# liuhx02/YourEditableAvatar

Hardware: AMD Instinct MI355X
Metric: rasterized fragments/sec (fwd+bwd) @500k Gaussians 1080p (higher is better)
Workload: dtype f32

## Files before the change

youreditableavatar_amd/csrc/tgs_api.hip:

```cpp
#include "tgs_device.hpp"
#include "../../include/tgs_raster.h"
#include "../../include/tgs_raster_testing.h"

#include <cstdarg>
#include <cstdio>
#include <cstring>

namespace tgs {
void launch_preprocess_fwd(hipStream_t, const FwdIn&, const CamParams&, const GeomState&, const ImgState&);
void launch_preprocess_fwd_batch(hipStream_t, const FwdIn&, const FwdViews&);
void launch_scan(hipStream_t, const GeomState&, const ImgState&, uint32_t nblocks, uint32_t T, uint32_t sort_cap, unsigned long long r_capacity,
                 uint32_t tile_bound, uint32_t heavy_bound, uint32_t mid_bound, Meta* host_meta, int light);
void launch_bin_count(hipStream_t, int P, const GeomState&, const ImgState&, uint32_t gx, uint32_t T);
void launch_scatter(hipStream_t, int P, const GeomState&, const ImgState&, const BinState&, uint32_t gx, uint32_t T);
void launch_tile_sort(hipStream_t, const GeomState&, const ImgState&, const BinState&, uint32_t gx, uint32_t T, uint64_t r_bound, const Meta* m,
                      uint32_t sort_cap, uint32_t tile_bound, uint32_t heavy_bound, uint32_t mid_bound);
void launch_render_fwd(hipStream_t, const ImgState&, const BinState&, int W, int H, uint32_t gx, uint32_t T, const Meta* m, const float* bg,
                       float* out_color, uint32_t tile_bound, uint32_t mid_bound, int light);
void launch_mark_visible(hipStream_t, int P, const float* means3D, const float* view, uint8_t* present);
void launch_alpha(hipStream_t, const ImgState&, size_t N, float* out_alpha);
void launch_render_bwd(hipStream_t, const ImgState&, const BinState&, int W, int H, uint32_t gx, uint32_t tiles, const float* bg, const float* dL_dpix,
                       const float* dL_dalpha, bool deterministic, uint32_t mid_tiles, int light, uint32_t T);
void launch_preprocess_bwd(hipStream_t, const BwdIn&, const CamParams&, const GeomState&, const BinState&);
void launch_preprocess_bwd_batch(hipStream_t, const BwdIn&, const BatchViews&);
// ... 906 lines not shown

int tgs_mark_visible(void* stream, int P, const float* means3D, const float* viewmatrix, const float* projmatrix, uint8_t* present)
{
    hipStream_t st = (hipStream_t)stream;
    g_err[0] = 0;
    (void)projmatrix;
    if (P == 0) return TGS_OK;
    if (P < 0 || !means3D || !viewmatrix || !present) return fail(TGS_ERR_INVALID, "bad arguments");
    launch_mark_visible(st, P, means3D, viewmatrix, present);
    hipError_t e = hipGetLastError();
    if (e != hipSuccess) return fail(TGS_ERR_HIP, "mark_visible: %s", hipGetErrorString(e));
    return TGS_OK;
}

int64_t tgs_state_field(void* stream, const char* field, int P, int width, int height, int64_t R, int has_sh, int has_scale_rot,
                        const void* geom_buffer, const void* binning_buffer, const void* img_buffer, void* dst, size_t dst_bytes)
{
    hipStream_t st = (hipStream_t)stream;
    g_err[0] = 0;
    const ViewArgs v{nullptr, width, height, nullptr, nullptr, nullptr, 0.f, 0.f};
    const size_t N = v.N(), T = v.T();
    const FrameBuffers fb = carve_frame(GeomShape{(size_t)P, has_sh != 0, has_scale_rot != 0}, v, R, geom_buffer, binning_buffer, img_buffer);
    const GeomState& g = fb.g; const ImgState& s = fb.s; const BinState& b = fb.b;
    const void* src = nullptr; size_t count = 0, esz = 4, stride = 0, rows = 0;
    if (!strcmp(field, "n_contrib")) { src = s.n_contrib; count = N; }
    else if (!strcmp(field, "final_T")) { src = s.final_T; count = N; }
    else if (!strcmp(field, "ranges")) { src = s.ranges; count = 2 * T; }
    else if (!strcmp(field, "means2D")) { src = g.pack; count = 2 * (size_t)P; esz = 8; stride = 64; rows = (size_t)P; }
    else if (!strcmp(field, "depths")) { src = g.depth; count = (size_t)P; }
    else if (!strcmp(field, "conic_opacity")) { src = (const char*)g.pack + 8; count = 4 * (size_t)P; esz = 16; stride = 64; rows = (size_t)P; }
    else if (!strcmp(field, "rgb")) { src = (const char*)g.pack + 24; count = 3 * (size_t)P; esz = 12; stride = 64; rows = (size_t)P; }
    else if (!strcmp(field, "tiles_touched")) { src = g.tiles_touched; count = (size_t)P; }
    else if (!strcmp(field, "tile_order")) { src = s.tile_order; count = T; }
    else if (!strcmp(field, "stamps")) { src = s.stamps; count = 8 * T; esz = 8; }
    else if (!strcmp(field, "block_masks")) { src = (const char*)b.recC + 4; count = (size_t)R; esz = 4; stride = 8; rows = (size_t)R; }
    else if (!strcmp(field, "quad_masks")) { src = b.qmask; count = (size_t)R; esz = 8; }
    else if (!strcmp(field, "point_list")) { src = b.keys; count = (size_t)R; esz = 4; stride = 8; rows = (size_t)R; }
    else return fail(TGS_ERR_INVALID, "unknown field %s", field);
    const size_t total = stride ? rows * esz : count * esz;
    if (dst_bytes < total) return fail(TGS_ERR_INVALID, "dst too small for %s", field);
    if (count == 0) return 0;
    if (stride) HIP_TRY(hipMemcpy2DAsync(dst, esz, src, stride, esz, rows, hipMemcpyDeviceToDevice, st));
    else HIP_TRY(hipMemcpyAsync(dst, src, total, hipMemcpyDeviceToDevice, st));
    return (int64_t)count;
}

}
```

youreditableavatar_amd/csrc/tgs_device.hpp:

```cpp
#pragma once
#include <hip/hip_runtime.h>
#include <cstdlib>
#include <stddef.h>
#include <stdint.h>

namespace tgs {

constexpr int TILE = 16;
constexpr int TILE_PIX = TILE * TILE;
constexpr int WAVE = 64;
constexpr int PRE_BLOCK = 256;
constexpr uint32_t SORT_LDS_CAP = 8192;
constexpr int COOP_TILES = 64;
constexpr int RANK_TILES = 4;
constexpr int SLAB_ROW = 3;
#ifndef TGS_BIN_WGS_MAX
#define TGS_BIN_WGS_MAX 256
#endif
constexpr int BIN_WGS_MAX = TGS_BIN_WGS_MAX;
constexpr int BIN_THREADS = 1024;
constexpr uint32_t BIN_LDS_TILES = 24576;

struct Meta {
    unsigned long long R;
    uint32_t max_count;
    uint32_t n_overflow;
    uint32_t error;
    uint32_t n_nonempty;
    uint32_t n_heavy;
    uint32_t n_mid;
    uint32_t pad[8];
};

constexpr uint32_t META_ERR_CAPACITY = 2u;
constexpr uint32_t META_ERR_TILE_BOUND = 4u;

struct ScanAux {
    uint32_t hist[40];
    uint32_t cursor[40];
    uint32_t done;
    uint32_t pad[47];
};
static_assert(sizeof(ScanAux) == 512, "ScanAux: 128 words, cleared by the first 128 threads of a block");

struct GeomState {
    float4* pack;
    uint2* live;
    float* depth;
    uint8_t* clamped;
    ushort4* rect;
    uint32_t* tiles_touched;
    uint32_t* offsets;
    uint32_t* block_sums;
    uint32_t* block_flags;
};
struct ImgState {
    Meta* meta;
    ScanAux* aux;
    uint2* ranges;
    uint32_t* tile_count;
    uint32_t* bin_table;
    uint32_t* ovf_tiles;
    uint32_t* tile_order;
    uint4* tile_desc;
    uint4* light_desc;
    float* final_T;
    uint32_t* n_contrib;
    unsigned long long* stamps;
};
struct BinState {
    unsigned long long* keys;
    uint32_t* tile_of;
    float4* recA;
    float4* recB;
    float2* recC;
    uint32_t* slot;
    uint2* qmask;
    float4* slab;
};

template <typename T>
__host__ __device__ inline void carve(char*& p, T*& out, size_t count)
{
    uintptr_t a = (reinterpret_cast<uintptr_t>(p) + 255) & ~uintptr_t(255);
    out = reinterpret_cast<T*>(a);
    p = reinterpret_cast<char*>(out + count);
}
__host__ __device__ inline size_t n_blocks(size_t P) { return (P + PRE_BLOCK - 1) / PRE_BLOCK; }

__host__ __device__ inline size_t geom_carve(GeomState& g, char* base, size_t P, bool has_sh, bool has_scale_rot)
{
    char* p = base;
    (void)has_sh; (void)has_scale_rot;
    carve(p, g.pack, 4 * P); carve(p, g.live, P); carve(p, g.depth, P);
    carve(p, g.clamped, P); carve(p, g.rect, P); carve(p, g.tiles_touched, P); carve(p, g.offsets, P);
    carve(p, g.block_sums, n_blocks(P) + 1); carve(p, g.block_flags, n_blocks(P) + 1);
    return (size_t)(p - base) + 256;
}
__host__ __device__ inline size_t img_carve(ImgState& s, char* base, size_t N, size_t T)
{
    char* p = base;
    carve(p, s.meta, 1); carve(p, s.aux, 1); carve(p, s.ranges, T); carve(p, s.tile_count, T); carve(p, s.bin_table, (size_t)BIN_WGS_MAX * T);
    carve(p, s.ovf_tiles, T); carve(p, s.tile_order, T); carve(p, s.tile_desc, T); carve(p, s.light_desc, T);
    carve(p, s.final_T, N); carve(p, s.n_contrib, N);
    carve(p, s.stamps, 8 * T);
    return (size_t)(p - base) + 256;
}
__host__ __device__ inline size_t bin_carve(BinState& b, char* base, size_t R)
{
    char* p = base;
    carve(p, b.keys, R); carve(p, b.tile_of, R); carve(p, b.recA, R); carve(p, b.recB, R); carve(p, b.recC, R); carve(p, b.slot, R); carve(p, b.qmask, R); carve(p, b.slab, (size_t)SLAB_ROW * R);
    return (size_t)(p - base) + 256;
}

int set_error(int code, const char* msg);
int hip_status(const char* what);

#ifdef __HIPCC__
#define TGS_DPP_ADD(v, ctrl, rowmask)                                                                      \
    v += __builtin_bit_cast(float, __builtin_amdgcn_update_dpp(0, __builtin_bit_cast(int, v), ctrl, rowmask, 0xf, false))

__device__ __forceinline__ float wave_sum(float v)
{
    TGS_DPP_ADD(v, 0xB1, 0xf);
    TGS_DPP_ADD(v, 0x4E, 0xf);
    TGS_DPP_ADD(v, 0x141, 0xf);
    TGS_DPP_ADD(v, 0x140, 0xf);
    TGS_DPP_ADD(v, 0x142, 0xa);
    TGS_DPP_ADD(v, 0x143, 0xc);
// ... 706 lines not shown
```

youreditableavatar_amd/csrc/tgs_forward.hip:

```cpp
#include "tgs_device.hpp"

namespace tgs {

__device__ __forceinline__ float conic_min_on_edge(float dfix, float lo, float hi, float Pfix, float Pvar, float B, float mB_over_Pvar)
{
    const float t = fminf(hi, fmaxf(lo, dfix * mB_over_Pvar));
    return 0.5f * (Pfix * dfix * dfix + Pvar * t * t) + B * dfix * t;
}

__device__ __forceinline__ unsigned long long quadrant_mask(float2 xy, float4 co, uint32_t tx, uint32_t ty)
{
    const float o255 = 255.0f * co.w;
    if (o255 < 0.999f) return 0ull;
    const float tau = (fmaxf(__logf(o255), 0.f) + 0.01f) * 1.001f;
    const float A = co.x, B = co.y, Cc = co.z;
    const float det = A * Cc - B * B;
    if (!(det > 0.f && A > 0.f && Cc > 0.f)) return ~0ull;
    const float rA = __builtin_amdgcn_rcpf(A), K = 2.f * A * tau, sl = -B * rA;
    const float ox = xy.x - (float)(tx * TILE), y0 = (float)(ty * TILE) - xy.y;
    uint32_t keep[2] = {0u, 0u};
#pragma unroll
    for (int R = 0; R < 8; R++) {
        const float dy0 = y0 + (float)(2 * R), dy1 = y0 + (float)(2 * R + 1);
        const float d0 = fmaf(-det * dy0, dy0, K), d1 = fmaf(-det * dy1, dy1, K);
        const float w0 = fmaf(__builtin_amdgcn_sqrtf(d0), rA, 0.01f), w1 = fmaf(__builtin_amdgcn_sqrtf(d1), rA, 0.01f);
        const float c0 = fmaf(sl, dy0, ox), c1 = fmaf(sl, dy1, ox);
        const float lo = fmaxf(fminf(c0 - w0, c1 - w1), 0.f), hi = fminf(fmaxf(c0 + w0, c1 + w1), 15.f);
        const int il = (int)ceilf(lo), ih = (int)floorf(hi);
        const uint32_t ql = (uint32_t)il >> 1, qh = (uint32_t)ih >> 1;
        const uint32_t m8 = (2u << qh) - (1u << ql);
        const bool some = !(fmaxf(d0, d1) < 0.f) && il <= ih;
        keep[R >> 2] |= (some ? m8 : 0u) << (8 * (R & 3));
    }
// ... 90 lines not shown
                        SH_C3_6 * x * (xx - 3.0f * yy) * SH(15);
                }
            }
        }
#undef SH
        r += 0.5f;
        if (r < 0.f) clampbits |= 1u << c;
        res[c] = fmaxf(r, 0.0f);
    }
    col0 = res[0]; col1 = res[1]; col2 = res[2];
}

struct PreColor { bool valid; float c0, c1, c2; uint32_t clampbits; };

struct GaussIn { float mx, my, mz, s0, s1, s2, opac; tgs_v4f q; };
template <bool HAS_SCALE_ROT>
__device__ __forceinline__ GaussIn load_gauss_in(const FwdIn& in, int idx)
{
    const size_t ic = idx < in.P ? (size_t)idx : 0;
    GaussIn gi;
    gi.mx = in.means3D[3 * ic]; gi.my = in.means3D[3 * ic + 1]; gi.mz = in.means3D[3 * ic + 2];
    gi.opac = in.opacities[ic];
    gi.s0 = gi.s1 = gi.s2 = 0.f; gi.q = tgs_v4f{0.f, 0.f, 0.f, 0.f};
    if (HAS_SCALE_ROT) {
        gi.s0 = in.scales[3 * ic]; gi.s1 = in.scales[3 * ic + 1]; gi.s2 = in.scales[3 * ic + 2];
        gi.q = reinterpret_cast<const tgs_v4f*>(in.rotations)[ic];
    }
    return gi;
}

template <bool HAS_SH, bool HAS_SCALE_ROT>
__device__ __forceinline__ uint32_t preprocess_fwd_one(const FwdIn& in, int* __restrict__ radii, const CamParams& cam, const GeomState& g, const ImgState& s,
                                                       const float4* sh_lds, bool sh_staged, int idx, const GaussIn& gi, const PreColor& pre, bool& prefilter_violation,
                                                       ReachTab& rtab)
{
#pragma clang fp contract(off)
    uint32_t tiles = 0;
    const ViewMat V = load_mat(cam.view), PM = load_mat(cam.proj);
    const float camx = cam.campos[0], camy = cam.campos[1], camz = cam.campos[2];
    int my_radius_i = 0;
    uint32_t minx = 0, miny = 0, maxx = 0, maxy = 0;
    bool have = false, mid = false;
    float pix = 0.f, piy = 0.f, conx = 0.f, cony = 0.f, conz = 0.f, opac = 0.f, col0 = 0.f, col1 = 0.f, col2 = 0.f;
    unsigned long long live_mask = 0ull;
    if (idx < in.P) {
        const float mx = gi.mx, my = gi.my, mz = gi.mz;
        const float* pm = PM.m;
        const float hx = pm[0] * mx + pm[4] * my + pm[8] * mz + pm[12];
        const float hy = pm[1] * mx + pm[5] * my + pm[9] * mz + pm[13];
        const float hw = pm[3] * mx + pm[7] * my + pm[11] * mz + pm[15];
        const float p_w = 1.0f / (hw + 0.0000001f);
        const float projx = hx * p_w, projy = hy * p_w;
        const float* vm = V.m;
        const float view_z = vm[2] * mx + vm[6] * my + vm[10] * mz + vm[14];
        bool ok = !(view_z <= 0.2f);
        prefilter_violation = !ok && in.prefiltered;
        if (ok) {
            float cov3d[6];
            if (HAS_SCALE_ROT) {
                compute_cov3d(cam.scale_modifier, gi.s0, gi.s1, gi.s2, make_float4(gi.q.x, gi.q.y, gi.q.z, gi.q.w), cov3d);
            } else {
#pragma unroll
                for (int i = 0; i < 6; i++) cov3d[i] = in.cov3D_precomp[6 * (size_t)idx + i];
            }
            const Cov2D c2 = compute_cov2d(mx, my, mz, cov3d, cam, V);
            const float cx = c2.cov.m[0][0] + 0.3f, cy = c2.cov.m[0][1], cz = c2.cov.m[1][1] + 0.3f;
            const float det = (cx * cz - cy * cy);
// ... 42 lines not shown
#pragma unroll
                        for (int k = 0; k < RANK_TILES; k++) {
                            if ((uint32_t)k < tiles) {
                                if (!in.prune || tile_reachable(make_float2(pix, piy), make_float4(conx, cony, conz, opac), minx + kx, miny + ky)) live_mask |= 1ull << k;
                                if (++kx == maxx - minx) { kx = 0; ky++; }
                            }
                        }
                        tiles = (uint32_t)__builtin_popcountll(live_mask);
                    } else if (tiles <= (uint32_t)COOP_TILES) {
                        if (in.prune) mid = true;
                        else live_mask = tiles >= 64u ? ~0ull : (1ull << tiles) - 1ull;
                    }
                }
            }
        }
    }
    if (__builtin_amdgcn_ballot_w64(mid) != 0ull) {
        const unsigned long long lm = wave_live_masks(mid, tiles, make_float2(pix, piy), make_float4(conx, cony, conz, opac), minx, miny, maxx - minx, rtab, threadIdx.x & 63);
        if (mid) { live_mask = lm; tiles = (uint32_t)__builtin_popcountll(lm); }
    }
    if (have) {
        float4* pk = g.pack + 4 * (size_t)idx;
        pk[0] = make_float4(pix, piy, conx, cony);
        pk[1] = make_float4(conz, opac, col0, col1);
        pk[2] = make_float4(col2, __uint_as_float(minx | (miny << 16)), __uint_as_float(maxx | (maxy << 16)), 0.f);
        pk[3] = make_float4(__uint_as_float((uint32_t)live_mask), __uint_as_float((uint32_t)(live_mask >> 32)), 0.f, 0.f);
        g.live[idx] = make_uint2((uint32_t)live_mask, (uint32_t)(live_mask >> 32));
    }
    if (idx < in.P) {
        if (radii) radii[idx] = my_radius_i;
        g.tiles_touched[idx] = tiles;
        g.rect[idx] = make_ushort4((unsigned short)minx, (unsigned short)miny, (unsigned short)maxx, (unsigned short)maxy);
    }
    return tiles;
}

__device__ __forceinline__ void block_sum_tiles(uint32_t tiles, bool violation, const GeomState& g, const ImgState& s)
{
    __shared__ uint32_t wsum[PRE_BLOCK / WAVE];
    __shared__ uint32_t wflag[PRE_BLOCK / WAVE];
    const uint32_t w = wave_sum_u32(tiles);
    const bool any = __builtin_amdgcn_ballot_w64(violation) != 0ull;
    if ((threadIdx.x & 63) == 0) { wsum[threadIdx.x >> 6] = w; wflag[threadIdx.x >> 6] = any ? 1u : 0u; }
    __syncthreads();
    if (threadIdx.x == 0) {
        g.block_sums[blockIdx.x] = wsum[0] + wsum[1] + wsum[2] + wsum[3];
        g.block_flags[blockIdx.x] = wflag[0] | wflag[1] | wflag[2] | wflag[3];
    }
    if (blockIdx.x == 0 && threadIdx.x < sizeof(Meta) / sizeof(uint32_t)) reinterpret_cast<uint32_t*>(s.meta)[threadIdx.x] = 0u;
    if (blockIdx.x == 0 && threadIdx.x < sizeof(ScanAux) / sizeof(uint32_t)) reinterpret_cast<uint32_t*>(s.aux)[threadIdx.x] = 0u;
}

__device__ __forceinline__ void stage_sh_rows(const FwdIn& in, float4* sh_lds)
{
    const float4* s4 = reinterpret_cast<const float4*>(in.shs);
    const size_t base4 = (size_t)blockIdx.x * PRE_BLOCK * 12, total4 = (size_t)in.P * 12;
    float4 r[12];
#pragma unroll
    for (int q = 0; q < 12; q++) { const size_t i = base4 + q * PRE_BLOCK + threadIdx.x; r[q] = nt_load4(&s4[i < total4 ? i : total4 - 1]); }
#pragma unroll
    for (int q = 0; q < 12; q++) sh_lds[q * PRE_BLOCK + threadIdx.x] = r[q];
    __syncthreads();
}

constexpr int SH_HALF = PRE_BLOCK / 2;
template <int NV>
__device__ __forceinline__ void sh_colors_half_staged(const FwdIn& in, const FwdView* __restrict__ views, int idx, const GaussIn& gi, float4* sh_lds, PreColor (&pre)[NV])
{
    const float4* s4 = reinterpret_cast<const float4*>(in.shs);
    const size_t base4 = (size_t)blockIdx.x * PRE_BLOCK * 12, total4 = (size_t)in.P * 12;
    constexpr int PER = SH_HALF * 12 / PRE_BLOCK;
    float4 r0[PER], r1[PER];
#pragma unroll
    for (int q = 0; q < PER; q++) { const size_t i = base4 + q * PRE_BLOCK + threadIdx.x; r0[q] = nt_load4(&s4[i < total4 ? i : total4 - 1]); }
#pragma unroll
    for (int q = 0; q < PER; q++) { const size_t i = base4 + SH_HALF * 12 + q * PRE_BLOCK + threadIdx.x; r1[q] = nt_load4(&s4[i < total4 ? i : total4 - 1]); }
#pragma unroll
    for (int q = 0; q < PER; q++) sh_lds[q * PRE_BLOCK + threadIdx.x] = r0[q];
    const float mx = gi.mx, my = gi.my, mz = gi.mz;
    auto eval = [&]() {
// ... 4 lines not shown
        for (int q = 0; q < 12; q++) {
            if (q * 4 < ncoef * 3) { const float4 t = row[q]; shv[4 * q] = t.x; shv[4 * q + 1] = t.y; shv[4 * q + 2] = t.z; shv[4 * q + 3] = t.w; }
        }
#pragma unroll
        for (int v = 0; v < NV; v++) {
            const CamParams& cam = views[v].cam;
            const float view_z = cam.view[2] * mx + cam.view[6] * my + cam.view[10] * mz + cam.view[14];
            pre[v].valid = true;
            if (!(view_z <= 0.2f)) sh_to_color(in.D, shv, mx - cam.campos[0], my - cam.campos[1], mz - cam.campos[2], pre[v].c0, pre[v].c1, pre[v].c2, pre[v].clampbits);
        }
    };
#pragma unroll
    for (int v = 0; v < NV; v++) { pre[v].valid = true; pre[v].c0 = pre[v].c1 = pre[v].c2 = 0.f; pre[v].clampbits = 0u; }
    __syncthreads();
    if (threadIdx.x < SH_HALF && idx < in.P) eval();
    __syncthreads();
#pragma unroll
    for (int q = 0; q < PER; q++) sh_lds[q * PRE_BLOCK + threadIdx.x] = r1[q];
    __syncthreads();
    if (threadIdx.x >= SH_HALF && idx < in.P) eval();
}

template <bool HAS_SH, bool HAS_SCALE_ROT>
__global__ __launch_bounds__(PRE_BLOCK) void k_preprocess_fwd(const FwdIn in, const FwdView vw)
{
    const int idx = blockIdx.x * PRE_BLOCK + threadIdx.x;
    __shared__ float4 sh_lds[HAS_SH ? SH_HALF * 12 : 1];
    __shared__ ReachTab rtab[PRE_BLOCK / WAVE];
    PreColor pre[1];
    pre[0].valid = false;
    const GaussIn gi = load_gauss_in<HAS_SCALE_ROT>(in, idx);
    if (HAS_SH && in.M == 16) sh_colors_half_staged<1>(in, &vw, idx, gi, sh_lds, pre);
    bool bad = false;
    const uint32_t tiles = preprocess_fwd_one<HAS_SH, HAS_SCALE_ROT>(in, vw.radii, vw.cam, vw.g, vw.s, sh_lds, false, idx, gi, pre[0], bad, rtab[threadIdx.x >> 6]);
    block_sum_tiles(tiles, bad, vw.g, vw.s);
}

template <bool HAS_SH, bool HAS_SCALE_ROT>
__global__ __launch_bounds__(PRE_BLOCK) void k_preprocess_fwd_pair(const FwdIn in, const FwdView v0, const FwdView v1)
{
    const int idx = blockIdx.x * PRE_BLOCK + threadIdx.x;
    __shared__ float4 sh_lds[HAS_SH ? SH_HALF * 12 : 1];
    __shared__ ReachTab rtab[PRE_BLOCK / WAVE];
    const FwdView vws[2] = {v0, v1};
    PreColor pre[2];
    pre[0].valid = pre[1].valid = false;
    const GaussIn gi = load_gauss_in<HAS_SCALE_ROT>(in, idx);
    if (HAS_SH && in.M == 16) sh_colors_half_staged<2>(in, vws, idx, gi, sh_lds, pre);
#pragma unroll
    for (int v = 0; v < 2; v++) {
        const FwdView& vw = v == 0 ? v0 : v1;
        bool bad = false;
        const uint32_t tiles = preprocess_fwd_one<HAS_SH, HAS_SCALE_ROT>(in, vw.radii, vw.cam, vw.g, vw.s, sh_lds, false, idx, gi, pre[v], bad, rtab[threadIdx.x >> 6]);
        block_sum_tiles(tiles, bad, vw.g, vw.s);
        __syncthreads();
    }
}

template <bool HAS_SH, bool HAS_SCALE_ROT>
__global__ __launch_bounds__(PRE_BLOCK) void k_preprocess_fwd_batch(const FwdIn in, const FwdViews views)
{
    const int idx = blockIdx.x * PRE_BLOCK + threadIdx.x;
    __shared__ float4 sh_lds[HAS_SH ? PRE_BLOCK * 12 : 1];
    __shared__ ReachTab rtab[PRE_BLOCK / WAVE];
    const bool sh_staged = HAS_SH && in.M == 16;
    const GaussIn gi = load_gauss_in<HAS_SCALE_ROT>(in, idx);
    if (sh_staged) stage_sh_rows(in, sh_lds);
    PreColor pre;
    pre.valid = false;
#pragma unroll 1
    for (int v = 0; v < views.n; v++) {
        const FwdView& vw = views.v[v];
        bool bad = false;
        const uint32_t tiles = preprocess_fwd_one<HAS_SH, HAS_SCALE_ROT>(in, vw.radii, vw.cam, vw.g, vw.s, sh_lds, sh_staged, idx, gi, pre, bad, rtab[threadIdx.x >> 6]);
        block_sum_tiles(tiles, bad, vw.g, vw.s);
        __syncthreads();
    }
}

constexpr int SCAN_THREADS = 1024;
constexpr int SCAN_ITEMS = 4;

__device__ __forceinline__ unsigned long long block_exscan_u64(unsigned long long v, unsigned long long* lds, unsigned long long& total)
{
    const int lane = threadIdx.x & 63, wv = threadIdx.x >> 6;
    const unsigned long long inc = wave_iscan_u64(v, lane);
    if (lane == 63) lds[wv] = inc;
    __syncthreads();
    unsigned long long base = 0, tot = 0;
#pragma unroll
    for (int i = 0; i < SCAN_THREADS / WAVE; i++) { const unsigned long long t = lds[i]; if (i < wv) base += t; tot += t; }
    __syncthreads();
    total = tot;
    return base + inc - v;
}
__device__ __forceinline__ uint32_t length_bucket(uint32_t n) { return n ? 32u - (uint32_t)__builtin_clz(n) : 0u; }

__global__ __launch_bounds__(SCAN_THREADS) void k_scan(const GeomState g, const ImgState s, uint32_t nblocks, uint32_t T, uint32_t sort_cap, unsigned long long r_capacity, uint32_t tile_bound,
                                                       uint32_t heavy_bound, uint32_t mid_bound, Meta* host_meta, int light)
{
    __shared__ unsigned long long lds[SCAN_THREADS / WAVE];
    __shared__ uint32_t lds_max[SCAN_THREADS / WAVE];
    if (blockIdx.x == 0) {
        unsigned long long carry = 0;
        uint32_t flags = 0;
        for (uint32_t base = 0; base < nblocks; base += SCAN_THREADS * SCAN_ITEMS) {
            uint32_t v[SCAN_ITEMS];
            unsigned long long sum = 0;
// ... 101 lines not shown
    }
    const uint32_t mid_area = (area > (uint32_t)EMIT_RANK && area <= (uint32_t)COOP_TILES) ? area : 0u;
    const uint32_t incl = wave_iscan_u32(mid_area, lane), total = (uint32_t)__builtin_amdgcn_readlane((int)incl, 63);
    if (total > 0) {
        tab.excl[lane] = incl - mid_area;
        tab.rect[lane] = make_uint2((uint32_t)r.x | ((uint32_t)r.y << 16), rw);
        tab.live[lane] = live;
        tab.key[lane] = key;
        wave_sync();
        for (uint32_t w = lane; w < total; w += 64) {
            uint32_t lo = 0, hi = 63;
#pragma unroll
            for (int it = 0; it < 6; it++) { const uint32_t mid = (lo + hi + 1) >> 1; if (tab.excl[mid] <= w) lo = mid; else hi = mid - 1; }
            const uint2 rc = tab.rect[lo];
            const uint32_t k = w - tab.excl[lo], rw2 = rc.y;
            if (!((tab.live[lo] >> k) & 1ull)) continue;
            const uint32_t ky = k / rw2;
            f(((rc.x >> 16) + ky) * gx + (rc.x & 0xffffu) + (k - ky * rw2), tab.key[lo]);
        }
        wave_sync();
    }
    unsigned long long bigs = __builtin_amdgcn_ballot_w64(area > (uint32_t)COOP_TILES);
    while (bigs) {
        const int src = __builtin_ctzll(bigs);
        bigs &= bigs - 1;
        const uint32_t x0 = (uint32_t)__builtin_amdgcn_readlane((int)r.x, src), y0 = (uint32_t)__builtin_amdgcn_readlane((int)r.y, src);
        const uint32_t w2 = (uint32_t)__builtin_amdgcn_readlane((int)rw, src), n = (uint32_t)__builtin_amdgcn_readlane((int)area, src);
        const unsigned long long kk = ((unsigned long long)(uint32_t)__builtin_amdgcn_readlane((int)(key >> 32), src) << 32) |
                                      (uint32_t)__builtin_amdgcn_readlane((int)(uint32_t)key, src);
        for (uint32_t k = lane; k < n; k += 64) { const uint32_t ky = k / w2; f((y0 + ky) * gx + x0 + (k - ky * w2), kk); }
    }
}

__global__ __launch_bounds__(BIN_THREADS) void k_bin_count(int P, uint32_t chunk, const GeomState g, const ImgState s, uint32_t gx, uint32_t T, uint32_t band)
{
    extern __shared__ uint32_t bin_lds[];
    __shared__ MidTab tabs[BIN_THREADS / WAVE];
    const int lane = threadIdx.x & 63, wv = threadIdx.x >> 6;
    const uint32_t lo = blockIdx.x * chunk;
    uint32_t* row = s.bin_table + (size_t)blockIdx.x * T;
    for (uint32_t band0 = 0; band0 < T; band0 += band) {
        const uint32_t nb = min(band, T - band0);
        for (uint32_t i = threadIdx.x; i < nb; i += BIN_THREADS) bin_lds[i] = 0u;
        __syncthreads();
        uint32_t n_tiles = 0; ushort4 n_r = make_ushort4(0, 0, 0, 0); uint2 n_live = make_uint2(0u, 0u);
        auto fetch = [&](uint32_t idx) {
            if (idx < (uint32_t)P) { n_tiles = g.tiles_touched[idx]; n_r = g.rect[idx]; n_live = g.live[idx]; } else n_tiles = 0u;
        };
        fetch(lo + threadIdx.x);
#pragma unroll 1
        for (uint32_t base = lo; base < lo + chunk; base += BIN_THREADS) {
            const uint32_t tiles = n_tiles; const ushort4 r = n_r; const uint2 live = n_live;
            if (base + BIN_THREADS < lo + chunk) fetch(base + BIN_THREADS + threadIdx.x);
            wave_emit_instances(tiles, r, live, 0ull, gx, tabs[wv], lane, [&](uint32_t t, unsigned long long) {
                if (t - band0 < nb) atomicAdd(&bin_lds[t - band0], 1u);
            });
        }
        __syncthreads();
        for (uint32_t i = threadIdx.x; i < nb; i += BIN_THREADS) row[band0 + i] = bin_lds[i];
        __syncthreads();
    }
}

constexpr int COL_WAVES = BIN_WGS_MAX / 32;
__global__ __launch_bounds__(64 * COL_WAVES) void k_bin_colscan(const ImgState s, uint32_t T, uint32_t nchunks)
{
    __shared__ uint32_t part[COL_WAVES][WAVE];
    __shared__ uint32_t bh[34];
    const int q = threadIdx.x >> 6, l = threadIdx.x & 63;
    if (threadIdx.x < 34) bh[threadIdx.x] = 0u;
    const uint32_t t = blockIdx.x * WAVE + l;
    const uint32_t per = (nchunks + COL_WAVES - 1) / COL_WAVES, w0 = min(nchunks, q * per), w1 = min(nchunks, w0 + per);
    uint32_t* col = s.bin_table + t;
    uint32_t c[BIN_WGS_MAX / COL_WAVES];
    uint32_t sum = 0;
    if (t < T) {
#pragma unroll
        for (int k = 0; k < BIN_WGS_MAX / COL_WAVES; k++) { c[k] = w0 + k < w1 ? col[(size_t)(w0 + k) * T] : 0u; }
#pragma unroll
        for (int k = 0; k < BIN_WGS_MAX / COL_WAVES; k++) sum += c[k];
    }
    part[q][l] = sum;
    __syncthreads();
    if (t < T) {
        uint32_t run = 0;
        for (int i = 0; i < q; i++) run += part[i][l];
#pragma unroll
        for (int k = 0; k < BIN_WGS_MAX / COL_WAVES; k++) { if (w0 + k < w1) col[(size_t)(w0 + k) * T] = run; run += c[k]; }
        if (q == COL_WAVES - 1) {
            s.tile_count[t] = run;
            atomicAdd(&bh[length_bucket(run)], 1u);
        }
    }
    __syncthreads();
    if (threadIdx.x < 34 && bh[threadIdx.x]) atomicAdd(&s.aux->hist[threadIdx.x], bh[threadIdx.x]);
}

#ifndef TGS_SCATTER_XCD_MAJOR
#define TGS_SCATTER_XCD_MAJOR 1
#endif
__device__ __forceinline__ uint32_t xcd_major(uint32_t b, uint32_t n)
{
    const uint32_t x = b & 7u, q = n >> 3, r = n & 7u;
    return x * q + min(x, r) + (b >> 3);
}
__global__ __launch_bounds__(BIN_THREADS) void k_scatter(int P, uint32_t chunk, const GeomState g, const ImgState s, const BinState b, uint32_t gx, uint32_t T, uint32_t band)
{
    extern __shared__ uint32_t bin_lds[];
    __shared__ MidTab tabs[BIN_THREADS / WAVE];
    __shared__ uint32_t wtot[2][BIN_THREADS / WAVE];
    const int lane = threadIdx.x & 63, wv = threadIdx.x >> 6;
    if (frame_rejected(s)) return;
    const uint32_t w = TGS_SCATTER_XCD_MAJOR ? xcd_major(blockIdx.x, gridDim.x) : blockIdx.x;
    const uint32_t lo = w * chunk;
    const uint32_t* row = s.bin_table + (size_t)w * T;
    for (uint32_t band0 = 0; band0 < T; band0 += band) {
        const uint32_t nb = min(band, T - band0);
        for (uint32_t i0 = threadIdx.x; i0 < nb; i0 += 8 * BIN_THREADS) {
            uint32_t st[8], cu[8];
#pragma unroll
            for (int u = 0; u < 8; u++) { const uint32_t ic = min(i0 + u * BIN_THREADS, nb - 1u); st[u] = s.ranges[band0 + ic].x; cu[u] = row[band0 + ic]; }
#pragma unroll
            for (int u = 0; u < 8; u++) { const uint32_t i = i0 + u * BIN_THREADS; if (i < nb) bin_lds[i] = st[u] + cu[u]; }
        }
        __syncthreads();
        int par = 0;
        uint32_t n_tiles = 0, n_depth = 0, n_bsum = 0; ushort4 n_r = make_ushort4(0, 0, 0, 0); uint2 n_live = make_uint2(0u, 0u);
        auto fetch = [&](uint32_t idx) {
            if (idx < (uint32_t)P) { n_tiles = g.tiles_touched[idx]; n_r = g.rect[idx]; n_live = g.live[idx]; n_depth = __float_as_uint(g.depth[idx]); n_bsum = g.block_sums[idx / PRE_BLOCK]; }
            else n_tiles = 0u;
        };
        fetch(lo + threadIdx.x);
#pragma unroll 1
        for (uint32_t base = lo; base < lo + chunk; base += BIN_THREADS, par ^= 1) {
            const uint32_t idx = base + threadIdx.x;
            const uint32_t tiles = n_tiles, bsum = n_bsum; const ushort4 r = n_r; const uint2 live = n_live;
            const unsigned long long key = ((unsigned long long)n_depth << 32) | idx;
            if (base + BIN_THREADS < lo + chunk) fetch(base + BIN_THREADS + threadIdx.x);
            if (band0 == 0) {
                const uint32_t inc = wave_iscan_u32(tiles, lane);
                if (lane == 63) wtot[par][wv] = inc;
                __syncthreads();
                if (idx < (uint32_t)P) {
                    uint32_t off = bsum + inc - tiles;
                    for (int i = wv & ~3; i < wv; i++) off += wtot[par][i];
                    g.offsets[idx] = off;
                    if (tiles > 0) reinterpret_cast<uint32_t*>(g.pack + 4 * (size_t)idx + 2)[3] = off;
                }
            }
            wave_emit_instances(tiles, r, live, key, gx, tabs[wv], lane, [&](uint32_t t, unsigned long long k) {
                if (t - band0 < nb) b.keys[atomicAdd(&bin_lds[t - band0], 1u)] = k;
            });
        }
        __syncthreads();
    }
}



template <int NT>
__device__ __forceinline__ void sort_tile_lds(unsigned long long* lk, uint32_t tid, uint32_t n, uint32_t npad_loop)
{
    const uint32_t half = npad_loop >> 1;
    const uint32_t lane = tid & 63, wv = tid >> 6;
    constexpr uint32_t W = NT / 64;
    for (uint32_t c = wv * SORT_CHUNK; c < n; c += W * SORT_CHUNK) {
        unsigned long long k0, k1;
        regs_load_chunk(lk, c, n, lane, k0, k1);
        regs_sort128(k0, k1, lane);
        regs_store_chunk(lk, c, n, lane, k0, k1);
    }
    __syncthreads();
    for (uint32_t k = 2 * SORT_CHUNK; k <= npad_loop; k <<= 1) {
        for (uint32_t p = tid; p < half; p += NT) { uint32_t i, l; pair_flip(p, k, i, l); cmp_swap(lk, i, l, n); }
        __syncthreads();
        for (uint32_t j = k >> 2; j >= SORT_CHUNK; j >>= 1) {
            for (uint32_t p = tid; p < half; p += NT) { uint32_t i, l; pair_disperse(p, j, i, l); cmp_swap(lk, i, l, n); }
            __syncthreads();
        }
        for (uint32_t c = wv * SORT_CHUNK; c < n; c += W * SORT_CHUNK) {
            unsigned long long k0, k1;
            regs_load_chunk(lk, c, n, lane, k0, k1);
            regs_disperse_from64(k0, k1, lane);
// ... 436 lines not shown
void launch_preprocess_fwd(hipStream_t st, const FwdIn& in, const CamParams& cam, const GeomState& g, const ImgState& s)
{
    const dim3 grid((unsigned)n_blocks(in.P)), blk(PRE_BLOCK);
    const bool sh = in.colors_precomp == nullptr, sr = in.cov3D_precomp == nullptr;
    FwdView vw;
    vw.cam = cam; vw.g = g; vw.s = s; vw.radii = in.radii;
    if (sh && sr) hipLaunchKernelGGL((k_preprocess_fwd<true, true>), grid, blk, 0, st, in, vw);
    else if (sh) hipLaunchKernelGGL((k_preprocess_fwd<true, false>), grid, blk, 0, st, in, vw);
    else if (sr) hipLaunchKernelGGL((k_preprocess_fwd<false, true>), grid, blk, 0, st, in, vw);
    else hipLaunchKernelGGL((k_preprocess_fwd<false, false>), grid, blk, 0, st, in, vw);
}
void launch_preprocess_fwd_batch(hipStream_t st, const FwdIn& in, const FwdViews& views)
{
    const dim3 grid((unsigned)n_blocks(in.P)), blk(PRE_BLOCK);
    const bool sh = in.colors_precomp == nullptr, sr = in.cov3D_precomp == nullptr;
    if (views.n == 2) {
        if (sh && sr) hipLaunchKernelGGL((k_preprocess_fwd_pair<true, true>), grid, blk, 0, st, in, views.v[0], views.v[1]);
        else if (sh) hipLaunchKernelGGL((k_preprocess_fwd_pair<true, false>), grid, blk, 0, st, in, views.v[0], views.v[1]);
        else if (sr) hipLaunchKernelGGL((k_preprocess_fwd_pair<false, true>), grid, blk, 0, st, in, views.v[0], views.v[1]);
        else hipLaunchKernelGGL((k_preprocess_fwd_pair<false, false>), grid, blk, 0, st, in, views.v[0], views.v[1]);
        return;
    }
    if (sh && sr) hipLaunchKernelGGL((k_preprocess_fwd_batch<true, true>), grid, blk, 0, st, in, views);
    else if (sh) hipLaunchKernelGGL((k_preprocess_fwd_batch<true, false>), grid, blk, 0, st, in, views);
    else if (sr) hipLaunchKernelGGL((k_preprocess_fwd_batch<false, true>), grid, blk, 0, st, in, views);
    else hipLaunchKernelGGL((k_preprocess_fwd_batch<false, false>), grid, blk, 0, st, in, views);
}
void launch_scan(hipStream_t st, const GeomState& g, const ImgState& s, uint32_t nblocks, uint32_t T, uint32_t sort_cap, unsigned long long r_capacity,
                 uint32_t tile_bound, uint32_t heavy_bound, uint32_t mid_bound, Meta* host_meta, int light)
{
    hipLaunchKernelGGL(k_scan, dim3(1u + (T + SCAN_THREADS - 1) / SCAN_THREADS), dim3(SCAN_THREADS), 0, st, g, s, nblocks, T, sort_cap, r_capacity, tile_bound, heavy_bound, mid_bound,
                       host_meta, light);
}
void bin_shape(int P, uint32_t T, uint32_t& nchunks, uint32_t& chunk, uint32_t& band, size_t& lds)
{
    static const int bin_wgs = [] {
        const char* e = getenv("TGS_BIN_WGS");
        const int v = e ? atoi(e) : BIN_WGS_MAX;
        return v < 1 ? 1 : (v > BIN_WGS_MAX ? BIN_WGS_MAX : v);
    }();
    const uint32_t per = ((uint32_t)P + (uint32_t)bin_wgs - 1) / (uint32_t)bin_wgs;
    chunk = (per + BIN_THREADS - 1) / BIN_THREADS * BIN_THREADS;
    if (chunk == 0) chunk = BIN_THREADS;
    nchunks = ((uint32_t)P + chunk - 1) / chunk;
    band = T < BIN_LDS_TILES ? T : BIN_LDS_TILES;
    lds = (size_t)band * sizeof(uint32_t);
}
void launch_bin_count(hipStream_t st, int P, const GeomState& g, const ImgState& s, uint32_t gx, uint32_t T)
{
    uint32_t nchunks, chunk, band; size_t lds;
    bin_shape(P, T, nchunks, chunk, band, lds);
    if (lds > 32 * 1024) (void)hipFuncSetAttribute((const void*)k_bin_count, hipFuncAttributeMaxDynamicSharedMemorySize, (int)lds);
    hipLaunchKernelGGL(k_bin_count, dim3(nchunks), dim3(BIN_THREADS), lds, st, P, chunk, g, s, gx, T, band);
    hipLaunchKernelGGL(k_bin_colscan, dim3((T + WAVE - 1) / WAVE), dim3(64 * COL_WAVES), 0, st, s, T, nchunks);
}
void launch_scatter(hipStream_t st, int P, const GeomState& g, const ImgState& s, const BinState& b, uint32_t gx, uint32_t T)
{
    uint32_t nchunks, chunk, band; size_t lds;
    bin_shape(P, T, nchunks, chunk, band, lds);
    if (lds > 32 * 1024) (void)hipFuncSetAttribute((const void*)k_scatter, hipFuncAttributeMaxDynamicSharedMemorySize, (int)lds);
    hipLaunchKernelGGL(k_scatter, dim3(nchunks), dim3(BIN_THREADS), lds, st, P, chunk, g, s, b, gx, T, band);
}
static uint32_t host_next_pow2(uint32_t n) { uint32_t p = 1; while (p < n) p <<= 1; return p; }
void launch_tile_sort(hipStream_t st, const GeomState& g, const ImgState& s, const BinState& b, uint32_t gx, uint32_t T, uint64_t r_bound,
                      const Meta* m, uint32_t sort_cap, uint32_t tile_bound, uint32_t heavy_bound, uint32_t mid_bound)
{
    if (!m && tile_bound < T) T = tile_bound;
    const uint32_t max_count = m ? m->max_count : sort_cap;
    const uint32_t cap = max_count < sort_cap ? max_count : sort_cap;
    const size_t lds = (size_t)(cap ? cap : 1) * 8;
    const uint32_t nonempty = m ? m->n_nonempty : (uint32_t)(r_bound < T ? r_bound : T);
    uint32_t heavy = m ? m->n_heavy : (uint32_t)(r_bound / 1024 < T ? r_bound / 1024 : T);
    uint32_t mid = m ? m->n_mid : (uint32_t)(r_bound / 128 < T ? r_bound / 128 : T);
    if (!m && heavy > heavy_bound) heavy = heavy_bound;
    if (!m && mid > mid_bound) mid = mid_bound;
    if (heavy > nonempty) heavy = nonempty;
    if (mid < heavy) mid = heavy;
    if (mid > nonempty) mid = nonempty;
    const uint32_t small = m ? nonempty - mid : nonempty;
    {
        const uint32_t mid_only = m ? mid - heavy : mid;
        const uint32_t mid_blocks = (mid_only + 3) / 4, small_blocks = (small + 15) / 16;
        size_t bytes = 0;
        if (heavy > 0) bytes = lds;
        if (mid_blocks > 0 && bytes < 4 * 1024 * 8) bytes = 4 * 1024 * 8;
        if (small_blocks > 0 && bytes < 16 * SORT_CHUNK * 8) bytes = 16 * SORT_CHUNK * 8;
        const uint32_t ovf_blocks = (m && m->n_overflow == 0) ? 0u : OVF_WORKERS;
// ... 22 lines not shown
```

Baseline: 969,500.

## Restrict binning tables to the bounding window of touched tiles

Preprocess now reduces a per-block bounding box of touched tiles. Bin count reduces these into a global window, stores it in ScanAux, and counts only over window-local tile indices. Colscan and scatter then index the per-chunk bin table by window coordinates and skip tiles outside the window. This is meant to cut LDS band passes and bin-table traffic when the Gaussians cover only part of the frame. The cost is an extra reduction over block boxes in every bin_count workgroup and more index arithmetic.

```diff
diff --git a/youreditableavatar_amd/csrc/tgs_api.hip b/youreditableavatar_amd/csrc/tgs_api.hip
--- a/youreditableavatar_amd/csrc/tgs_api.hip
+++ b/youreditableavatar_amd/csrc/tgs_api.hip
@@ -962,6 +962,8 @@
     else if (!strcmp(field, "rgb")) { src = (const char*)g.pack + 24; count = 3 * (size_t)P; esz = 12; stride = 64; rows = (size_t)P; }
     else if (!strcmp(field, "tiles_touched")) { src = g.tiles_touched; count = (size_t)P; }
     else if (!strcmp(field, "tile_order")) { src = s.tile_order; count = T; }
+    else if (!strcmp(field, "tile_count")) { src = s.tile_count; count = T; }
+    else if (!strcmp(field, "offsets")) { src = g.offsets; count = (size_t)P; }
     else if (!strcmp(field, "stamps")) { src = s.stamps; count = 8 * T; esz = 8; }
     else if (!strcmp(field, "block_masks")) { src = (const char*)b.recC + 4; count = (size_t)R; esz = 4; stride = 8; rows = (size_t)R; }
     else if (!strcmp(field, "quad_masks")) { src = b.qmask; count = (size_t)R; esz = 8; }
diff --git a/youreditableavatar_amd/csrc/tgs_device.hpp b/youreditableavatar_amd/csrc/tgs_device.hpp
--- a/youreditableavatar_amd/csrc/tgs_device.hpp
+++ b/youreditableavatar_amd/csrc/tgs_device.hpp
@@ -39,8 +39,11 @@
     uint32_t hist[40];
     uint32_t cursor[40];
     uint32_t done;
-    uint32_t pad[47];
-};
+    uint32_t pad0[3];
+    uint32_t window[4];
+    uint32_t pad[40];
+};
+static_assert(offsetof(ScanAux, window) % 16 == 0, "ScanAux::window is stored and loaded as one 16-byte piece");
 static_assert(sizeof(ScanAux) == 512, "ScanAux: 128 words, cleared by the first 128 threads of a block");
 
 struct GeomState {
@@ -53,6 +56,7 @@
     uint32_t* offsets;
     uint32_t* block_sums;
     uint32_t* block_flags;
+    uint2* block_box;
 };
 struct ImgState {
     Meta* meta;
@@ -80,9 +84,9 @@
 };
 
 template <typename T>
-__host__ __device__ inline void carve(char*& p, T*& out, size_t count)
-{
-    uintptr_t a = (reinterpret_cast<uintptr_t>(p) + 255) & ~uintptr_t(255);
+__host__ __device__ inline void carve(char*& p, T*& out, size_t count, uintptr_t align = 256)
+{
+    uintptr_t a = (reinterpret_cast<uintptr_t>(p) + (align - 1)) & ~(align - 1);
     out = reinterpret_cast<T*>(a);
     p = reinterpret_cast<char*>(out + count);
 }
@@ -94,7 +98,8 @@
     (void)has_sh; (void)has_scale_rot;
     carve(p, g.pack, 4 * P); carve(p, g.live, P); carve(p, g.depth, P);
     carve(p, g.clamped, P); carve(p, g.rect, P); carve(p, g.tiles_touched, P); carve(p, g.offsets, P);
-    carve(p, g.block_sums, n_blocks(P) + 1); carve(p, g.block_flags, n_blocks(P) + 1);
+    carve(p, g.block_sums, n_blocks(P) + 1); carve(p, g.block_box, n_blocks(P) + 1, 16);
+    carve(p, g.block_flags, n_blocks(P) + 1);
     return (size_t)(p - base) + 256;
 }
 __host__ __device__ inline size_t img_carve(ImgState& s, char* base, size_t N, size_t T)
diff --git a/youreditableavatar_amd/csrc/tgs_forward.hip b/youreditableavatar_amd/csrc/tgs_forward.hip
--- a/youreditableavatar_amd/csrc/tgs_forward.hip
+++ b/youreditableavatar_amd/csrc/tgs_forward.hip
@@ -1,4 +1,5 @@
 #include "tgs_device.hpp"
+#include <atomic>
 
 namespace tgs {
 
@@ -155,7 +156,7 @@
 template <bool HAS_SH, bool HAS_SCALE_ROT>
 __device__ __forceinline__ uint32_t preprocess_fwd_one(const FwdIn& in, int* __restrict__ radii, const CamParams& cam, const GeomState& g, const ImgState& s,
                                                        const float4* sh_lds, bool sh_staged, int idx, const GaussIn& gi, const PreColor& pre, bool& prefilter_violation,
-                                                       ReachTab& rtab)
+                                                       ReachTab& rtab, uint2& box)
 {
 #pragma clang fp contract(off)
     uint32_t tiles = 0;
@@ -264,20 +265,31 @@
         g.tiles_touched[idx] = tiles;
         g.rect[idx] = make_ushort4((unsigned short)minx, (unsigned short)miny, (unsigned short)maxx, (unsigned short)maxy);
     }
+    box = tiles ? make_uint2((0xffffu - minx) | (maxx << 16), (0xffffu - miny) | (maxy << 16)) : make_uint2(0u, 0u);
     return tiles;
 }
 
-__device__ __forceinline__ void block_sum_tiles(uint32_t tiles, bool violation, const GeomState& g, const ImgState& s)
+__device__ __forceinline__ void block_sum_tiles(uint32_t tiles, uint2 box, bool violation, const GeomState& g, const ImgState& s)
 {
     __shared__ uint32_t wsum[PRE_BLOCK / WAVE];
     __shared__ uint32_t wflag[PRE_BLOCK / WAVE];
+    __shared__ uint32_t wbox[4][PRE_BLOCK / WAVE];
     const uint32_t w = wave_sum_u32(tiles);
     const bool any = __builtin_amdgcn_ballot_w64(violation) != 0ull;
-    if ((threadIdx.x & 63) == 0) { wsum[threadIdx.x >> 6] = w; wflag[threadIdx.x >> 6] = any ? 1u : 0u; }
+    const uint32_t b0 = wave_max_u32(box.x & 0xffffu), b1 = wave_max_u32(box.x >> 16), b2 = wave_max_u32(box.y & 0xffffu), b3 = wave_max_u32(box.y >> 16);
+    if ((threadIdx.x & 63) == 0) {
+        const int wv = threadIdx.x >> 6;
+        wsum[wv] = w; wflag[wv] = any ? 1u : 0u;
+        wbox[0][wv] = b0; wbox[1][wv] = b1; wbox[2][wv] = b2; wbox[3][wv] = b3;
+    }
     __syncthreads();
     if (threadIdx.x == 0) {
         g.block_sums[blockIdx.x] = wsum[0] + wsum[1] + wsum[2] + wsum[3];
         g.block_flags[blockIdx.x] = wflag[0] | wflag[1] | wflag[2] | wflag[3];
+        uint32_t m[4];
+#pragma unroll
+        for (int k = 0; k < 4; k++) m[k] = max(max(wbox[k][0], wbox[k][1]), max(wbox[k][2], wbox[k][3]));
+        g.block_box[blockIdx.x] = make_uint2(m[0] | (m[1] << 16), m[2] | (m[3] << 16));
     }
     if (blockIdx.x == 0 && threadIdx.x < sizeof(Meta) / sizeof(uint32_t)) reinterpret_cast<uint32_t*>(s.meta)[threadIdx.x] = 0u;
     if (blockIdx.x == 0 && threadIdx.x < sizeof(ScanAux) / sizeof(uint32_t)) reinterpret_cast<uint32_t*>(s.aux)[threadIdx.x] = 0u;
@@ -348,8 +360,9 @@
     const GaussIn gi = load_gauss_in<HAS_SCALE_ROT>(in, idx);
     if (HAS_SH && in.M == 16) sh_colors_half_staged<1>(in, &vw, idx, gi, sh_lds, pre);
     bool bad = false;
-    const uint32_t tiles = preprocess_fwd_one<HAS_SH, HAS_SCALE_ROT>(in, vw.radii, vw.cam, vw.g, vw.s, sh_lds, false, idx, gi, pre[0], bad, rtab[threadIdx.x >> 6]);
-    block_sum_tiles(tiles, bad, vw.g, vw.s);
+    uint2 box;
+    const uint32_t tiles = preprocess_fwd_one<HAS_SH, HAS_SCALE_ROT>(in, vw.radii, vw.cam, vw.g, vw.s, sh_lds, false, idx, gi, pre[0], bad, rtab[threadIdx.x >> 6], box);
+    block_sum_tiles(tiles, box, bad, vw.g, vw.s);
 }
 
 template <bool HAS_SH, bool HAS_SCALE_ROT>
@@ -367,8 +380,9 @@
     for (int v = 0; v < 2; v++) {
         const FwdView& vw = v == 0 ? v0 : v1;
         bool bad = false;
-        const uint32_t tiles = preprocess_fwd_one<HAS_SH, HAS_SCALE_ROT>(in, vw.radii, vw.cam, vw.g, vw.s, sh_lds, false, idx, gi, pre[v], bad, rtab[threadIdx.x >> 6]);
-        block_sum_tiles(tiles, bad, vw.g, vw.s);
+        uint2 box;
+        const uint32_t tiles = preprocess_fwd_one<HAS_SH, HAS_SCALE_ROT>(in, vw.radii, vw.cam, vw.g, vw.s, sh_lds, false, idx, gi, pre[v], bad, rtab[threadIdx.x >> 6], box);
+        block_sum_tiles(tiles, box, bad, vw.g, vw.s);
         __syncthreads();
     }
 }
@@ -388,8 +402,9 @@
     for (int v = 0; v < views.n; v++) {
         const FwdView& vw = views.v[v];
         bool bad = false;
-        const uint32_t tiles = preprocess_fwd_one<HAS_SH, HAS_SCALE_ROT>(in, vw.radii, vw.cam, vw.g, vw.s, sh_lds, sh_staged, idx, gi, pre, bad, rtab[threadIdx.x >> 6]);
-        block_sum_tiles(tiles, bad, vw.g, vw.s);
+        uint2 box;
+        const uint32_t tiles = preprocess_fwd_one<HAS_SH, HAS_SCALE_ROT>(in, vw.radii, vw.cam, vw.g, vw.s, sh_lds, sh_staged, idx, gi, pre, bad, rtab[threadIdx.x >> 6], box);
+        block_sum_tiles(tiles, box, bad, vw.g, vw.s);
         __syncthreads();
     }
 }
@@ -557,27 +572,68 @@
     }
 }
 
-__global__ __launch_bounds__(BIN_THREADS) void k_bin_count(int P, uint32_t chunk, const GeomState g, const ImgState s, uint32_t gx, uint32_t T, uint32_t band)
+#ifndef TGS_BIN_WINDOW
+#define TGS_BIN_WINDOW 1
+#endif
+struct BinWindow { uint32_t x0, y0, ww, wh; };
+__device__ __forceinline__ ushort4 window_rect(ushort4 r, const BinWindow& w)
+{
+    return make_ushort4((unsigned short)(r.x - w.x0), (unsigned short)(r.y - w.y0), (unsigned short)(r.z - w.x0), (unsigned short)(r.w - w.y0));
+}
+__device__ __forceinline__ BinWindow load_window(const ImgState& s)
+{
+    const tgs_v4f t = __builtin_nontemporal_load(reinterpret_cast<const tgs_v4f*>(s.aux->window));
+    return BinWindow{__float_as_uint(t.x), __float_as_uint(t.y), __float_as_uint(t.z), __float_as_uint(t.w)};
+}
+
+__global__ __launch_bounds__(BIN_THREADS) void k_bin_count(int P, uint32_t chunk, const GeomState g, const ImgState s, uint32_t gx, uint32_t T, uint32_t band, int whole_grid)
 {
     extern __shared__ uint32_t bin_lds[];
     __shared__ MidTab tabs[BIN_THREADS / WAVE];
+    __shared__ uint32_t wbox[4][BIN_THREADS / WAVE];
     const int lane = threadIdx.x & 63, wv = threadIdx.x >> 6;
     const uint32_t lo = blockIdx.x * chunk;
     uint32_t* row = s.bin_table + (size_t)blockIdx.x * T;
-    for (uint32_t band0 = 0; band0 < T; band0 += band) {
-        const uint32_t nb = min(band, T - band0);
+    uint32_t n_tiles = 0; ushort4 n_r = make_ushort4(0, 0, 0, 0); uint2 n_live = make_uint2(0u, 0u);
+    auto fetch = [&](uint32_t idx) {
+        if (idx < (uint32_t)P) { n_tiles = g.tiles_touched[idx]; n_r = g.rect[idx]; n_live = g.live[idx]; } else n_tiles = 0u;
+    };
+    uint32_t m0 = 0, m1 = 0, m2 = 0, m3 = 0;
+    const uint32_t nblk = (uint32_t)n_blocks((size_t)P);
+    for (uint32_t i = threadIdx.x; i < nblk; i += BIN_THREADS) {
+        const uint2 bx = g.block_box[i];
+        m0 = max(m0, bx.x & 0xffffu); m1 = max(m1, bx.x >> 16); m2 = max(m2, bx.y & 0xffffu); m3 = max(m3, bx.y >> 16);
+    }
+    fetch(lo + threadIdx.x);
+    m0 = wave_max_u32(m0); m1 = wave_max_u32(m1); m2 = wave_max_u32(m2); m3 = wave_max_u32(m3);
+    if (lane == 0) { wbox[0][wv] = m0; wbox[1][wv] = m1; wbox[2][wv] = m2; wbox[3][wv] = m3; }
+    __syncthreads();
+    m0 = m1 = m2 = m3 = 0;
+#pragma unroll
+    for (int i = 0; i < BIN_THREADS / WAVE; i++) { m0 = max(m0, wbox[0][i]); m1 = max(m1, wbox[1][i]); m2 = max(m2, wbox[2][i]); m3 = max(m3, wbox[3][i]); }
+    const uint32_t gy = T / gx;
+    BinWindow win;
+    {
+        const uint32_t x0 = 0xffffu - m0, x1 = min(m1, gx), y0 = 0xffffu - m2, y1 = min(m3, gy);
+        const bool some = x0 < x1 && y0 < y1;
+        win = some ? BinWindow{x0, y0, x1 - x0, y1 - y0} : BinWindow{0u, 0u, 0u, 0u};
+        if (!TGS_BIN_WINDOW || whole_grid) win = BinWindow{0u, 0u, gx, gy};
+    }
+    if (blockIdx.x == 0 && threadIdx.x == 0) {
+        tgs_v4f t; t.x = __uint_as_float(win.x0); t.y = __uint_as_float(win.y0); t.z = __uint_as_float(win.ww); t.w = __uint_as_float(win.wh);
+        *reinterpret_cast<tgs_v4f*>(s.aux->window) = t;
+    }
+    const uint32_t Tw = win.ww * win.wh;
+    for (uint32_t band0 = 0; band0 < Tw; band0 += band) {
+        const uint32_t nb = min(band, Tw - band0);
         for (uint32_t i = threadIdx.x; i < nb; i += BIN_THREADS) bin_lds[i] = 0u;
         __syncthreads();
-        uint32_t n_tiles = 0; ushort4 n_r = make_ushort4(0, 0, 0, 0); uint2 n_live = make_uint2(0u, 0u);
-        auto fetch = [&](uint32_t idx) {
-            if (idx < (uint32_t)P) { n_tiles = g.tiles_touched[idx]; n_r = g.rect[idx]; n_live = g.live[idx]; } else n_tiles = 0u;
-        };
-        fetch(lo + threadIdx.x);
+        if (band0 != 0) fetch(lo + threadIdx.x);
 #pragma unroll 1
         for (uint32_t base = lo; base < lo + chunk; base += BIN_THREADS) {
-            const uint32_t tiles = n_tiles; const ushort4 r = n_r; const uint2 live = n_live;
+            const uint32_t tiles = n_tiles; const ushort4 r = window_rect(n_r, win); const uint2 live = n_live;
             if (base + BIN_THREADS < lo + chunk) fetch(base + BIN_THREADS + threadIdx.x);
-            wave_emit_instances(tiles, r, live, 0ull, gx, tabs[wv], lane, [&](uint32_t t, unsigned long long) {
+            wave_emit_instances(tiles, r, live, 0ull, win.ww, tabs[wv], lane, [&](uint32_t t, unsigned long long) {
                 if (t - band0 < nb) atomicAdd(&bin_lds[t - band0], 1u);
             });
         }
@@ -588,18 +644,27 @@
 }
 
 constexpr int COL_WAVES = BIN_WGS_MAX / 32;
-__global__ __launch_bounds__(64 * COL_WAVES) void k_bin_colscan(const ImgState s, uint32_t T, uint32_t nchunks)
+__global__ __launch_bounds__(64 * COL_WAVES) void k_bin_colscan(const ImgState s, uint32_t gx, uint32_t T, uint32_t nchunks)
 {
     __shared__ uint32_t part[COL_WAVES][WAVE];
     __shared__ uint32_t bh[34];
     const int q = threadIdx.x >> 6, l = threadIdx.x & 63;
+    const BinWindow win = load_window(s);
     if (threadIdx.x < 34) bh[threadIdx.x] = 0u;
     const uint32_t t = blockIdx.x * WAVE + l;
+    const uint32_t ty = t / gx, tx = t - ty * gx;
+    const bool inw = t < T && tx - win.x0 < win.ww && ty - win.y0 < win.wh;
+    const unsigned long long inw_any = __builtin_amdgcn_ballot_w64(inw);
+    if (inw_any == 0ull) {
+        if (q == COL_WAVES - 1 && t < T) s.tile_count[t] = 0u;
+        if (threadIdx.x == 0) atomicAdd(&s.aux->hist[0], min((uint32_t)WAVE, T - blockIdx.x * WAVE));
+        return;
+    }
     const uint32_t per = (nchunks + COL_WAVES - 1) / COL_WAVES, w0 = min(nchunks, q * per), w1 = min(nchunks, w0 + per);
-    uint32_t* col = s.bin_table + t;
+    uint32_t* col = s.bin_table + ((ty - win.y0) * win.ww + (tx - win.x0));
     uint32_t c[BIN_WGS_MAX / COL_WAVES];
     uint32_t sum = 0;
-    if (t < T) {
+    if (inw) {
 #pragma unroll
         for (int k = 0; k < BIN_WGS_MAX / COL_WAVES; k++) { c[k] = w0 + k < w1 ? col[(size_t)(w0 + k) * T] : 0u; }
 #pragma unroll
@@ -607,7 +672,7 @@
     }
     part[q][l] = sum;
     __syncthreads();
-    if (t < T) {
+    if (inw) {
         uint32_t run = 0;
         for (int i = 0; i < q; i++) run += part[i][l];
 #pragma unroll
@@ -616,6 +681,9 @@
             s.tile_count[t] = run;
             atomicAdd(&bh[length_bucket(run)], 1u);
         }
+    } else if (t < T && q == COL_WAVES - 1) {
+        s.tile_count[t] = 0u;
+        atomicAdd(&bh[0], 1u);
     }
     __syncthreads();
     if (threadIdx.x < 34 && bh[threadIdx.x]) atomicAdd(&s.aux->hist[threadIdx.x], bh[threadIdx.x]);
@@ -635,16 +703,21 @@
     __shared__ MidTab tabs[BIN_THREADS / WAVE];
     __shared__ uint32_t wtot[2][BIN_THREADS / WAVE];
     const int lane = threadIdx.x & 63, wv = threadIdx.x >> 6;
+    const BinWindow win = load_window(s);
     if (frame_rejected(s)) return;
     const uint32_t w = TGS_SCATTER_XCD_MAJOR ? xcd_major(blockIdx.x, gridDim.x) : blockIdx.x;
     const uint32_t lo = w * chunk;
     const uint32_t* row = s.bin_table + (size_t)w * T;
-    for (uint32_t band0 = 0; band0 < T; band0 += band) {
-        const uint32_t nb = min(band, T - band0);
+    const uint32_t Tw = win.ww * win.wh;
+    for (uint32_t band0 = 0; band0 == 0 || band0 < Tw; band0 += band) {
+        const uint32_t nb = min(band, Tw - band0);
         for (uint32_t i0 = threadIdx.x; i0 < nb; i0 += 8 * BIN_THREADS) {
             uint32_t st[8], cu[8];
 #pragma unroll
-            for (int u = 0; u < 8; u++) { const uint32_t ic = min(i0 + u * BIN_THREADS, nb - 1u); st[u] = s.ranges[band0 + ic].x; cu[u] = row[band0 + ic]; }
+            for (int u = 0; u < 8; u++) {
+                const uint32_t ic = band0 + min(i0 + u * BIN_THREADS, nb - 1u), wy = ic / win.ww;
+                st[u] = s.ranges[(win.y0 + wy) * gx + win.x0 + (ic - wy * win.ww)].x; cu[u] = row[ic];
+            }
 #pragma unroll
             for (int u = 0; u < 8; u++) { const uint32_t i = i0 + u * BIN_THREADS; if (i < nb) bin_lds[i] = st[u] + cu[u]; }
         }
@@ -659,7 +732,7 @@
 #pragma unroll 1
         for (uint32_t base = lo; base < lo + chunk; base += BIN_THREADS, par ^= 1) {
             const uint32_t idx = base + threadIdx.x;
-            const uint32_t tiles = n_tiles, bsum = n_bsum; const ushort4 r = n_r; const uint2 live = n_live;
+            const uint32_t tiles = n_tiles, bsum = n_bsum; const ushort4 r = window_rect(n_r, win); const uint2 live = n_live;
             const unsigned long long key = ((unsigned long long)n_depth << 32) | idx;
             if (base + BIN_THREADS < lo + chunk) fetch(base + BIN_THREADS + threadIdx.x);
             if (band0 == 0) {
@@ -673,7 +746,7 @@
                     if (tiles > 0) reinterpret_cast<uint32_t*>(g.pack + 4 * (size_t)idx + 2)[3] = off;
                 }
             }
-            wave_emit_instances(tiles, r, live, key, gx, tabs[wv], lane, [&](uint32_t t, unsigned long long k) {
+            wave_emit_instances(tiles, r, live, key, win.ww, tabs[wv], lane, [&](uint32_t t, unsigned long long k) {
                 if (t - band0 < nb) b.keys[atomicAdd(&bin_lds[t - band0], 1u)] = k;
             });
         }
@@ -1176,6 +1249,10 @@
     hipLaunchKernelGGL(k_scan, dim3(1u + (T + SCAN_THREADS - 1) / SCAN_THREADS), dim3(SCAN_THREADS), 0, st, g, s, nblocks, T, sort_cap, r_capacity, tile_bound, heavy_bound, mid_bound,
                        host_meta, light);
 }
+static std::atomic<int> g_bin_window{TGS_BIN_WINDOW};
+static std::atomic<uint32_t> g_bin_band{BIN_LDS_TILES};
+extern "C" void tgs_set_bin_window(int on) { g_bin_window.store(on < 0 ? TGS_BIN_WINDOW : (on ? 1 : 0), std::memory_order_relaxed); }
+extern "C" void tgs_set_bin_band(unsigned tiles) { g_bin_band.store(tiles == 0 || tiles > BIN_LDS_TILES ? BIN_LDS_TILES : tiles, std::memory_order_relaxed); }
 void bin_shape(int P, uint32_t T, uint32_t& nchunks, uint32_t& chunk, uint32_t& band, size_t& lds)
 {
     static const int bin_wgs = [] {
@@ -1187,7 +1264,8 @@
     chunk = (per + BIN_THREADS - 1) / BIN_THREADS * BIN_THREADS;
     if (chunk == 0) chunk = BIN_THREADS;
     nchunks = ((uint32_t)P + chunk - 1) / chunk;
-    band = T < BIN_LDS_TILES ? T : BIN_LDS_TILES;
+    const uint32_t cap = g_bin_band.load(std::memory_order_relaxed);
+    band = T < cap ? T : cap;
     lds = (size_t)band * sizeof(uint32_t);
 }
 void launch_bin_count(hipStream_t st, int P, const GeomState& g, const ImgState& s, uint32_t gx, uint32_t T)
@@ -1195,8 +1273,8 @@
     uint32_t nchunks, chunk, band; size_t lds;
     bin_shape(P, T, nchunks, chunk, band, lds);
     if (lds > 32 * 1024) (void)hipFuncSetAttribute((const void*)k_bin_count, hipFuncAttributeMaxDynamicSharedMemorySize, (int)lds);
-    hipLaunchKernelGGL(k_bin_count, dim3(nchunks), dim3(BIN_THREADS), lds, st, P, chunk, g, s, gx, T, band);
-    hipLaunchKernelGGL(k_bin_colscan, dim3((T + WAVE - 1) / WAVE), dim3(64 * COL_WAVES), 0, st, s, T, nchunks);
+    hipLaunchKernelGGL(k_bin_count, dim3(nchunks), dim3(BIN_THREADS), lds, st, P, chunk, g, s, gx, T, band, g_bin_window.load(std::memory_order_relaxed) ? 0 : 1);
+    hipLaunchKernelGGL(k_bin_colscan, dim3((T + WAVE - 1) / WAVE), dim3(64 * COL_WAVES), 0, st, s, gx, T, nchunks);
 }
 void launch_scatter(hipStream_t st, int P, const GeomState& g, const ImgState& s, const BinState& b, uint32_t gx, uint32_t T)
 {
```

Result: no change. 967,700 (-0.2%).
